# Epist/omnidirectional_collaborative_filtering

Measured on AMD Instinct MI355X. Metric: ratings/sec + masked-RMSE, ML-20M I-AutoRec at 1/2/4/8 MI355X, higher is better.
Workload: dtype f16

## Files before the change

omnidirectional_collaborative_filtering_amd/csrc/ocf_gemm.hip:

```cpp
#include <algorithm>
#include <cstdlib>
#include <type_traits>

#include "ocf_epilogues.h"
#include "ocf_internal.h"
#include "ocf_optim_ws.h"
#include "ocf_rows.h"

using namespace ocf;

namespace {

template <typename CT, bool ACOL, bool BCOL, typename BGT, class Epi, bool SPA = false>
void launch(const OcfGemmArgs& g, const typename Epi::Params& ep, hipStream_t s) {
  using Cfg = GemmCfg<CT, ACOL, BCOL, CT, BGT>;
  constexpr int LDS = std::max(Cfg::OPER_LDS, Epi::LDS_NEED);
  static_assert(LDS <= 160 * 1024, "LDS budget");
  GemmShape sh;
  sh.A = g.A; sh.B = g.B; sh.lda = g.lda; sh.ldb = g.ldb;
  sh.M = g.M; sh.N = g.N; sh.K = g.K; sh.order = g.order;
  sh.a_nt = g.a_nt != 0; sh.b_nt = g.b_nt != 0;
  sh.b_blk = g.b_blocked != 0;
  if (sh.b_blk)
    OCF_CHECK(sizeof(BGT) == 2 && g.ldb % 64 == 0, "ocf_gemm: blocked B needs a 16-bit compute-dtype B and ldb % 64 == 0");
// ... 169 lines not shown
        OCF_CHECK(g.h_dtype == OCF_F32 || g.h_dtype == OCF_BF16, "ocf_gemm GRAD: fp32 or bf16 gradient output");
        EpiGradStore::Params p{g.out, g.ld_out, g.opt.gscale, g.h_dtype == OCF_BF16 ? 1 : 0};
        if constexpr (ACOL) {
          if (g.a_sparse) {
            launch<CT, ACOL, BCOL, CT, EpiGradStore, true>(g, p, s);
            return;
          }
        }
        launch<CT, ACOL, BCOL, CT, EpiGradStore>(g, p, s);
        return;
      }
      break;
    default:
      break;
  }
  throw std::runtime_error("ocf_gemm: epilogue " + std::to_string(g.epi) + " not instantiated for layout a_col=" +
                           std::to_string(ACOL) + " b_col=" + std::to_string(BCOL) + " b_dtype=" +
                           std::to_string(g.b_dtype));
}

template <typename CT, bool ACOL, bool BCOL>
void dispatch_layout(const OcfGemmArgs& g, hipStream_t s) {
  const bool weight_b = g.epi == OCF_EPI_SLAB || g.epi == OCF_EPI_BIAS_ACT || g.epi == OCF_EPI_PREDICT ||
                        g.epi == OCF_EPI_MASKED_MSE || g.epi == OCF_EPI_GRAD_ACT;
  if (weight_b && g.b_dtype == OCF_F32) return dispatch_epi<CT, ACOL, BCOL, float>(g, s);
  OCF_CHECK(g.b_dtype == g.compute_dtype, weight_b ? "ocf_gemm: weight B must be fp32 or the compute dtype"
                                                   : "ocf_gemm: OPTIM/GRAD take B in the compute dtype");
  dispatch_epi<CT, ACOL, BCOL, CT>(g, s);
}


template <typename CT>
void dispatch(const OcfGemmArgs& g, hipStream_t s) {
  if (!g.a_col && g.b_col) dispatch_layout<CT, false, true>(g, s);
  else if (!g.a_col && !g.b_col) dispatch_layout<CT, false, false>(g, s);
  else if (g.a_col && g.b_col) dispatch_layout<CT, true, true>(g, s);
  else throw std::runtime_error("ocf_gemm: layout A[K][M] x B[N][K] not instantiated");
}

}

extern "C" int ocf_set_tuning(const char* key, int value, int* previous) {
  OCF_TRY_BEGIN
  const std::string k = key ? key : "";
  if (k == "optim_rows") {
    if (previous) *previous = g_optim_rows;
    g_optim_rows = value ? 1 : 0;
  } else if (k == "rows_long") {
    if (previous) *previous = g_rows_long;
    g_rows_long = value < 0 ? -1 : (value ? 1 : 0);
  } else if (k == "rows_dual") {
    if (previous) *previous = g_rows_dual;
    g_rows_dual = value ? 1 : 0;
  } else if (k == "rows_dual_parts") {
    if (previous) *previous = g_rows_dual_parts;
    OCF_CHECK(value >= 0 && value <= 64, "ocf_set_tuning: rows_dual_parts 0 (by size) or 1..64");
    g_rows_dual_parts = value;
  } else if (k == "rows_dual_pf") {
    if (previous) *previous = g_rows_dual_pf;
    g_rows_dual_pf = value < 0 ? -1 : value ? 1 : 0;
  } else if (k == "rows_dual_large") {
    if (previous) *previous = g_rows_dual_large;
    g_rows_dual_large = value ? 1 : 0;
  } else if (k == "rows_dual_count") {
    if (previous) *previous = g_rows_dual_count;
    g_rows_dual_count = 0;
  } else if (k == "rows_small_waves") {
    if (previous) *previous = g_rows_small_waves;
    g_rows_small_waves = value;
  } else if (k == "optim_ws") {
    if (previous) *previous = optim_ws_on() ? 1 : 0;
    g_optim_ws = value ? 1 : 0;
  } else if (k == "pair_wait_polls") {
    if (previous) *previous = g_pair_wait_polls;
    OCF_CHECK(value > 0, "ocf_set_tuning: pair_wait_polls > 0");
    g_pair_wait_polls = value;
  } else if (k == "encdec_max_polls") {
    if (previous) *previous = g_encdec_max_polls;
    OCF_CHECK(value != 0, "ocf_set_tuning: encdec_max_polls != 0");
    g_encdec_max_polls = value;
  } else if (k == "encdec_rowres") {
    if (previous) *previous = g_encdec_rowres;
    if (value >= 0) g_encdec_rowres = value ? 1 : 0;
  } else if (k == "mlp_max_polls") {
    if (previous) *previous = g_mlp_max_polls;
    OCF_CHECK(value != 0, "ocf_set_tuning: mlp_max_polls != 0");
    g_mlp_max_polls = value;
  } else if (k == "enc_tiles_pack") {
    if (previous) *previous = g_enc_tiles_pack;
    g_enc_tiles_pack = value ? 1 : 0;
  } else if (k == "optim_ws_max_k") {
    if (previous) *previous = g_optim_ws_max_k;
    g_optim_ws_max_k = value;
  } else {
    throw std::runtime_error("ocf_set_tuning: unknown key '" + k + "'");
  }
  OCF_TRY_END
}

namespace {
void check_gemm(const OcfGemmArgs& g) {
  OCF_CHECK((g.A || g.a_sparse) && g.B, "ocf_gemm: null operand");
  OCF_CHECK(g.M > 0 && g.N > 0 && g.K > 0, "ocf_gemm: empty shape");
  OCF_CHECK(g.M % GT_BM == 0 && g.N % GT_BN == 0, "ocf_gemm: M and N must be multiples of 128");
  const int bk = g.compute_dtype == OCF_F32 ? 32 : 64;
  OCF_CHECK(g.K % bk == 0, "ocf_gemm: K must be a multiple of 64 (f16/bf16) or 32 (f32)");
  OCF_CHECK(g.a_dtype == g.compute_dtype, "ocf_gemm: A must be in the compute dtype");
  OCF_CHECK(g.lda % 8 == 0 && g.ldb % 8 == 0, "ocf_gemm: leading dimensions must be multiples of 8");
  OCF_CHECK(g.splits >= 1, "ocf_gemm: splits >= 1");
  OCF_CHECK(g.splits == 1 || g.epi == OCF_EPI_SLAB, "ocf_gemm: split-K only with the SLAB epilogue");
  if (g.a_sparse) {
    OCF_CHECK(g.a_col && (g.epi == OCF_EPI_OPTIM || g.epi == OCF_EPI_GRAD),
              "ocf_gemm: sparse A only for OPTIM / GRAD with a_col = 1");
    OCF_CHECK(g.sp_rows && g.sp_rp && g.sp_tptr && g.sp_col && g.sp_lidx && g.sp_lboff && g.sp_vals &&
                  g.sp_ntiles * GT_BM >= g.M && g.sp_krows <= g.K,
              "ocf_gemm: sparse A descriptor incomplete");
  }
  OCF_CHECK(!(g.cb_p || g.jb_part || g.js_sp) || (g.epi == OCF_EPI_OPTIM && g.a_col),
            "ocf_gemm: folded jobs only with OPTIM on [K][M] A");
  OCF_CHECK(!g.cb_p || g.sp_colsum, "ocf_gemm: cb_p needs sp_colsum");
  OCF_CHECK(!g.jb_part || g.jb_p, "ocf_gemm: jb_part needs jb_p");
  OCF_CHECK(!g.js_sp || g.js_out, "ocf_gemm: js_sp needs js_out");
}

}

extern "C" int ocf_gemm(const OcfGemmArgs* args, void* stream) {
  OCF_TRY_BEGIN
  const OcfGemmArgs& g = *args;
  check_gemm(g);
  hipStream_t s = (hipStream_t)stream;
  switch (g.compute_dtype) {
    case OCF_F16: dispatch<_Float16>(g, s); break;
    case OCF_BF16: dispatch<__bf16>(g, s); break;
    case OCF_F32: dispatch<float>(g, s); break;
    default: throw std::runtime_error("ocf_gemm: bad compute dtype");
  }
  OCF_TRY_END
}

extern "C" int ocf_gemm_pair(const OcfGemmArgs* a, const OcfGemmArgs* b, OcfPairSync* sync, void* stream) {
  OCF_TRY_BEGIN
  OCF_CHECK(a && b, "ocf_gemm_pair: null arguments");
  OCF_CHECK(!sync || sync->word, "ocf_gemm_pair: OcfPairSync without a device word");
  check_gemm(*a);
  check_gemm(*b);
  hipStream_t s = (hipStream_t)stream;
  bool done = false;
  if (sync && a->compute_dtype == b->compute_dtype) {
    switch (a->compute_dtype) {
      case OCF_F16: done = launch_rows_pair<_Float16>(*a, *b, *sync, s); break;
      case OCF_BF16: done = launch_rows_pair<__bf16>(*a, *b, *sync, s); break;
      case OCF_F32: done = launch_rows_pair<float>(*a, *b, *sync, s); break;
      default: break;
    }
  }
  if (!done) {
    OCF_CHECK(ocf_gemm(a, stream) == 0, ocf_last_error());
    OCF_CHECK(ocf_gemm(b, stream) == 0, ocf_last_error());
  }
  OCF_TRY_END
}

extern "C" int ocf_train_step_rows(const OcfRowStepArgs* a, void* stream) {
  OCF_TRY_BEGIN
  OCF_CHECK(a != nullptr, "ocf_train_step_rows: null arguments");
// ... 32 lines not shown
```

omnidirectional_collaborative_filtering_amd/csrc/ocf_internal.h:

```cpp
#pragma once
#include <exception>
#include <stdexcept>
#include <string>

#include "../../include/ocf.h"
#include "ocf_common.h"

namespace ocf {
using ScatterArgs = OcfScatterArgs;
void set_error(const std::string& msg);
uint32_t* async_error_word();
void check_async_errors();
extern int g_mlp_max_polls;
extern int g_encdec_max_polls;
extern int g_encdec_rowres;
bool rank_rowres_enc(const OcfGatherArgs& e, const OcfRowsReduceArgs& r, hipStream_t s);
bool rank_rowres_dec(const OcfBiasActArgs& hb, const OcfGatherArgs& d, const OcfRowsReduceArgs& r, hipStream_t s);
extern int g_enc_tiles_pack;
uint32_t* encdec_gate_word();
uint32_t encdec_generation();
uint32_t next_encdec_generation();
}

#define OCF_TRY_BEGIN try { ocf::check_async_errors();
#define OCF_TRY_END                                       \
  return 0;                                               \
  }                                                       \
  catch (const std::exception& e) {                       \
    ocf::set_error(e.what());                             \
    return 1;                                             \
  }

#define OCF_CHECK(cond, msg)                              \
  do {                                                    \
    if (!(cond)) throw std::runtime_error(msg);           \
  } while (0)

#define OCF_HIP(expr)                                                               \
  do {                                                                              \
    hipError_t _e = (expr);                                                         \
    if (_e != hipSuccess)                                                           \
      throw std::runtime_error(std::string("HIP error: ") + hipGetErrorString(_e) + \
                               " at " __FILE__ ":" + std::to_string(__LINE__));     \
  } while (0)
```

omnidirectional_collaborative_filtering_amd/csrc/ocf_sparse.hip:

```cpp
#include <algorithm>
#include <cstdlib>

#include "ocf_epilogues.h"
#include "ocf_internal.h"

namespace ocf {

#ifndef OCF_RG_THREADS
#define OCF_RG_THREADS 256
#endif
constexpr int RG_THREADS = OCF_RG_THREADS;
constexpr int RG_MAX_H = 512;
#ifndef OCF_RG_U
#define OCF_RG_U 4
#endif
constexpr int RG_U = OCF_RG_U;
#ifndef OCF_RG_UE
#define OCF_RG_UE 4
#endif
constexpr int RG_UE = OCF_RG_UE;
#ifndef OCF_RG_UD
#define OCF_RG_UD 4
#endif
constexpr int RG_UD = OCF_RG_UD;
// ... 364 lines not shown
        float f[E];
        unpack_piece<WT>(w[u][i], f);
#pragma unroll
        for (int k = 0; k < E; ++k) d0 += hv[i * E + k] * f[k];
      }
      dot[u] = d0;
    }
#pragma unroll
    for (int off = G / 2; off > 0; off >>= 1)
#pragma unroll
      for (int u = 0; u < RG_UD; ++u) dot[u] += __shfl_xor(dot[u], off, G);
#pragma unroll
    for (int u = 0; u < RG_UD; ++u) {
      const int ju = j + u * NG;
      if (ju >= j1) break;
      float d = 0.f;
      if (lv[u]) {
        const float yh = m * (dot[u] + bn[u]);
        const float err = yh - tc[u];
        d = err * m;
        if (l == 0) {
          sse += err * err;
          sae += fabsf(err);
          cnt += (tc[u] + yh != 0.f) ? 1.f : 0.f;
          if (a.d_out) store_ct(a.d_out, a.d_dtype, (int64_t)b * a.ld_d + nc[u], d);
        }
      }
      if (l == 0 && a.delta_e) a.delta_e[lb + ju] = d;
#pragma unroll
      for (int i = 0; i < PPL; ++i) {
        float f[E];
        unpack_piece<WT>(w[u][i], f);
#pragma unroll
        for (int k = 0; k < E; ++k) acc[i * E + k] += d * f[k];
      }
    }
  }
  if (l == 0) {
    st[grp][0] = sse;
    st[grp][1] = sae;
    st[grp][2] = cnt;
  }
  const bool solo = fold && jr.row_cptr[b + 1] - jr.row_cptr[b] == 1;
  float own[RG_XPT];
  reduce_groups<G, V, E, PPL>(acc, red, a.part, c, a.H, grp, l, fold, solo, own);
  float own_st = 0.f;
  if (threadIdx.x < 3) {
    float v = 0.f;
    for (int g = 0; g < NG; ++g) v += st[g][threadIdx.x];
    own_st = v;
    if (solo) {
    } else if (fold) {
      st_sc1(a.chunk_stats, (int64_t)c * 4 + threadIdx.x, v);
    } else {
      a.chunk_stats[(int64_t)c * 4 + threadIdx.x] = v;
    }
  }
  if (fold) dec_row_tail(a, jr, b, a_sh, mk_sh, a.enc_part != nullptr, solo, own, own_st, enc_arrive);
}

template <typename WT, typename HT, int G, int PPL>
__global__ void __launch_bounds__(RG_THREADS) gather_decoder_kernel(OcfGatherArgs a, OcfRowsReduceArgs jr) {
  __shared__ float red[(RG_THREADS / G) * RG_MAX_H];
  decoder_chunk<WT, HT, G, PPL>(a, jr, blockIdx.x, blockIdx.x == 0, red, EncDecSync{});
}

template <typename WT, typename HT, int G, int PPL>
__global__ void __launch_bounds__(RG_THREADS) gather_encdec_kernel(OcfGatherArgs e, OcfGatherArgs d,
                                                                   OcfRowsReduceArgs jr, EncDecSync sy) {
  __shared__ float red[(RG_THREADS / G) * RG_MAX_H];
  const int bx = blockIdx.x;
  if (bx < e.n_chunks) encoder_chunk<WT, G, PPL, RG_UE>(e, bx, red, sy.enc_arrive);
  else decoder_chunk<WT, HT, G, PPL>(d, jr, bx - e.n_chunks, bx == e.n_chunks, red, sy);
}

#ifndef OCF_RR_UD
#define OCF_RR_UD 2
#endif
#ifndef OCF_RR_UE
#define OCF_RR_UE 4
#endif
constexpr int RR_UE = OCF_RR_UE;
constexpr int RR_UD = OCF_RR_UD;

enum { RR_FULL = 0,
       RR_ENC_RAW = 1,
       RR_DEC_RAW = 2 };

template <int G, int V, int E, int PPL>
__device__ __forceinline__ void rr_wave_sums(float (&acc)[V], float (*red)[RG_MAX_H], int l, int lane, int w) {
#pragma unroll
  for (int off = G; off < 64; off <<= 1)
#pragma unroll
    for (int k = 0; k < V; ++k) acc[k] += __shfl_xor(acc[k], off, 64);
  if (lane < G) {
#pragma unroll
    for (int i = 0; i < PPL; ++i)
#pragma unroll
      for (int k = 0; k < E; ++k) red[w][(l + G * i) * E + k] = acc[i * E + k];
  }
}
__device__ __forceinline__ void rr_lds_barrier() { asm volatile("s_waitcnt lgkmcnt(0)\n\ts_barrier" ::: "memory"); }
template <int NW>
__device__ __forceinline__ float rr_row_sum(const float (*red)[RG_MAX_H], int x) {
  float s0 = 0.f, s1 = 0.f;
#pragma unroll
  for (int w = 0; w < NW; w += 2) {
    s0 += red[w][x];
    s1 += red[w + 1][x];
  }
  return s0 + s1;
}
__device__ __forceinline__ float rr_sum_slabs(const float* s, int splits, int64_t sstride) {
  float v0 = 0.f, v1 = 0.f, v2 = 0.f, v3 = 0.f;
  int k = 0;
  for (; k + 4 <= splits; k += 4) {
    v0 += s[(int64_t)(k + 0) * sstride];
    v1 += s[(int64_t)(k + 1) * sstride];
    v2 += s[(int64_t)(k + 2) * sstride];
    v3 += s[(int64_t)(k + 3) * sstride];
  }
  for (; k < splits; ++k) v0 += s[(int64_t)k * sstride];
  return (v0 + v1) + (v2 + v3);
}

template <typename WT, typename HT, int G, int PPL, int T, int MODE>
__global__ void __launch_bounds__(T) gather_rowres_kernel(OcfGatherArgs e, OcfGatherArgs d, OcfRowsReduceArgs r,
                                                          OcfBiasActArgs hb) {
  constexpr int E = EPc<WT>::v;
  constexpr int V = PPL * E;
  constexpr int NG = T / G;
  constexpr int NW = T / 64;
  constexpr int XPT = (RG_MAX_H + T - 1) / T;
  __shared__ float red[NW][RG_MAX_H];
  __shared__ float h_sh[RG_MAX_H];
  __shared__ float a_sh[RG_MAX_H];
  __shared__ uint8_t mk_sh[RG_MAX_H];
  __shared__ float st_sh[NG][3];
  const int b = blockIdx.x, tid = threadIdx.x, lane = tid & 63, w = tid >> 6;
  const int grp = tid / G, l = tid % G;
  const OcfGatherArgs& q = MODE == RR_ENC_RAW ? e : d;
  const int H = q.H;
  const int64_t rb = (int64_t)b * H;
  if (MODE == RR_FULL && d.zero_word && b == 0 && tid == 0)
    __hip_atomic_store(d.zero_word, 0ull, __ATOMIC_RELAXED, __HIP_MEMORY_SCOPE_AGENT);
  const int row = b < r.B ? q.rows[b] : -1;
  const int64_t lb = b < r.B ? q.lboff[b] : 0;
  const int n_e = row >= 0 ? (int)(q.lboff[b + 1] - lb) : 0;
  if (n_e == 0 && MODE != RR_DEC_RAW) {
    for (int x = tid; x < H; x += T) {
      if (MODE == RR_FULL) {
        store_ct(r.h_out, r.h_dtype, rb + x, 0.f);
        if (r.db_part) r.db_part[rb + x] = 0.f;
      } else {
        r.out[rb + x] = 0.f;
      }
    }
    if (MODE == RR_FULL) {
      if (tid < 4) r.stats_part[(int64_t)b * 4 + tid] = 0.f;
      if (tid == 0 && r.row_sse) r.row_sse[b] = 0.f;
    }
    return;
  }
  const int64_t s = n_e > 0 ? q.rp[row] : 0;
  if constexpr (MODE != RR_DEC_RAW) {
    const WT* W = reinterpret_cast<const WT*>(e.W);
// ... 131 lines not shown
        tc[u] = t[u];
      }
      idx_d(j + NG * RR_UD);
      float dot[RR_UD];
#pragma unroll
      for (int u = 0; u < RR_UD; ++u) dot[u] = 0.f;
#pragma unroll
      for (int i = 0; i < PPL; ++i) {
        float hh[E];
#pragma unroll
        for (int k = 0; k < E; ++k) hh[k] = h_sh[(l + G * i) * E + k];
#pragma unroll
        for (int u = 0; u < RR_UD; ++u) {
          float f[E];
          unpack_piece<WT>(wv[u][i], f);
#pragma unroll
          for (int k = 0; k < E; ++k) dot[u] += hh[k] * f[k];
        }
      }
#pragma unroll
      for (int off = G / 2; off > 0; off >>= 1)
#pragma unroll
        for (int u = 0; u < RR_UD; ++u) dot[u] += __shfl_xor(dot[u], off, G);
#pragma unroll
      for (int u = 0; u < RR_UD; ++u) {
        const int ju = j + u * NG;
        if (ju >= n_e) break;
        float dl = 0.f;
        if (lv[u]) {
          const float yh = m * (dot[u] + bn[u]);
          const float err = yh - tc[u];
          dl = err * m;
          if (l == 0) {
            sse += err * err;
            sae += fabsf(err);
            cnt += (tc[u] + yh != 0.f) ? 1.f : 0.f;
            if (d.d_out) store_ct(d.d_out, d.d_dtype, (int64_t)b * d.ld_d + nc[u], dl);
          }
        }
        if (l == 0 && d.delta_e) d.delta_e[lb + ju] = dl;
#pragma unroll
        for (int i = 0; i < PPL; ++i) {
          float f[E];
          unpack_piece<WT>(wv[u][i], f);
#pragma unroll
          for (int k = 0; k < E; ++k) acc[i * E + k] += dl * f[k];
        }
      }
      load_d();
    }
    if (l == 0) {
      st_sh[grp][0] = sse;
      st_sh[grp][1] = sae;
      st_sh[grp][2] = cnt;
    }
    __syncthreads();
    rr_wave_sums<G, V, E, PPL>(acc, red, l, lane, w);
  }
  __syncthreads();
  for (int x = tid; x < H; x += T) {
    const float v = rr_row_sum<NW>(red, x);
    if constexpr (MODE == RR_DEC_RAW) {
      r.out[rb + x] = v;
    } else {
      float dv = 0.f;
      if (x < r.n_real) {
        dv = v;
        if (r.keep < 1.f && r.mask_in) dv = dv * ((float)mk_sh[x] / r.keep);
        dv = dv * act_grad(r.act, a_sh[x]);
      }
      store_ct(r.h_out, r.h_dtype, rb + x, dv);
      if (r.db_part) r.db_part[rb + x] = dv * r.gscale;
    }
  }
  if (tid < 4) {
    float v = 0.f;
    if (tid < 3)
      for (int g = 0; g < NG; ++g) v += st_sh[g][tid];
    r.stats_part[(int64_t)b * 4 + tid] = v;
    if (tid == 0 && r.row_sse) r.row_sse[b] = v;
  }
}

__global__ void __launch_bounds__(256) rows_reduce_kernel(OcfRowsReduceArgs a) {
  const int b = blockIdx.x;
  const bool real = b < a.B;
  const int c0 = real ? a.row_cptr[b] : 0, c1 = real ? a.row_cptr[b + 1] : 0;
  for (int x = threadIdx.x; x < a.H; x += blockDim.x) {
    float v = 0.f;
    for (int c = c0; c < c1; c += 8) {
      float q[8];
#pragma unroll
      for (int k = 0; k < 8; ++k) q[k] = c + k < c1 ? a.part[(int64_t)(c + k) * a.H + x] : 0.f;
#pragma unroll
      for (int k = 0; k < 8; ++k)
        if (c + k < c1) v += q[k];
    }
    if (a.mode == OCF_REDUCE_RAW) {
      a.out[(int64_t)b * a.H + x] = v;
    } else if (a.mode == OCF_REDUCE_BIAS_ACT) {
      BiasActParams p;
      p.bias = a.bias; p.act = a.act; p.keep = a.keep; p.seed = a.seed; p.stream = a.stream;
      p.mask_in = a.mask_in; p.mask_out = a.mask_out; p.a_out = a.a_out; p.h_out = a.h_out;
      p.h_dtype = a.h_dtype; p.ld = a.H; p.m_real = a.B; p.n_real = a.n_real;
      bias_act_store(p, b, x, v);
    } else {
      GradActParams p;
      p.a = a.a_in; p.mask = a.mask_in; p.keep = a.keep; p.act = a.act; p.d_out = a.h_out; p.d_dtype = a.h_dtype;
      p.ld = a.H; p.db_part = nullptr; p.gscale = a.gscale; p.m_real = a.B; p.n_real = a.n_real;
      const float d = grad_act_value(p, b, x, v);
      store_ct(a.h_out, a.h_dtype, (int64_t)b * a.H + x, d);
      if (a.db_part) a.db_part[(int64_t)b * a.H + x] = d * a.gscale;
    }
  }
  if (a.chunk_stats && threadIdx.x < 4) {
    float v = 0.f;
    if (threadIdx.x < 3)
      for (int c = c0; c < c1; c += 8) {
        float q[8];
#pragma unroll
        for (int k = 0; k < 8; ++k) q[k] = c + k < c1 ? a.chunk_stats[(int64_t)(c + k) * 4 + threadIdx.x] : 0.f;
#pragma unroll
        for (int k = 0; k < 8; ++k)
          if (c + k < c1) v += q[k];
      }
    a.stats_part[(int64_t)b * 4 + threadIdx.x] = v;
    if (threadIdx.x == 0 && a.row_sse) a.row_sse[b] = v;
  }
}

template <typename WT> bool gather_shape(int H, int& G, int& ppl) {
  const int pieces = H / EPc<WT>::v;
  constexpr int gmax = 32;
  for (int g : {64, 32, 16})
    if (g <= gmax && pieces % g == 0 && pieces / g <= 4) {
      G = g;
      ppl = pieces / g;
      return true;
    }
  for (int g : {64, 32, 16})
    if (pieces % g == 0) {
      G = g;
      ppl = pieces / g;
      return ppl <= 3;
    }
  return false;
}

template <template <int, int> class L>
void by_shape(int G, int ppl, const OcfGatherArgs& a, hipStream_t s) {
  if (G == 64 && ppl == 1) L<64, 1>::go(a, s);
  else if (G == 64 && ppl == 2) L<64, 2>::go(a, s);
  else if (G == 32 && ppl == 1) L<32, 1>::go(a, s);
  else if (G == 32 && ppl == 2) L<32, 2>::go(a, s);
  else if (G == 16 && ppl == 4) L<16, 4>::go(a, s);
  else if (G == 32 && ppl == 4) L<32, 4>::go(a, s);
  else if (G == 32 && ppl == 3) L<32, 3>::go(a, s);
  else if (G == 16 && ppl == 1) L<16, 1>::go(a, s);
  else if (G == 16 && ppl == 3) L<16, 3>::go(a, s);
  else throw std::runtime_error("row gather: unsupported H / weight dtype combination");
}

template <typename WT> struct Enc {
  template <int G, int P> struct L {
    static void go(const OcfGatherArgs& a, hipStream_t s) {
      hipLaunchKernelGGL((gather_encoder_kernel<WT, G, P>), dim3(a.n_chunks), dim3(RG_THREADS), 0, s, a);
    }
  };
};
template <typename WT, typename HT> struct Dec {
  template <int G, int P> struct L {
    static void go(const OcfGatherArgs& a, hipStream_t s) {
      OcfRowsReduceArgs r{};
      if (a.jr && a.row_arrive) r = *a.jr;
      hipLaunchKernelGGL((gather_decoder_kernel<WT, HT, G, P>), dim3(a.n_chunks), dim3(RG_THREADS), 0, s, a, r);
    }
  };
};

template <typename WT, typename HT>
void launch_encdec(int G, int ppl, const OcfGatherArgs& e, const OcfGatherArgs& d, const EncDecSync& sy, hipStream_t s) {
  OcfRowsReduceArgs r = *d.jr;
  const dim3 grid(e.n_chunks + d.n_chunks), blk(RG_THREADS);
#define OCF_ED(GG, PP) hipLaunchKernelGGL((gather_encdec_kernel<WT, HT, GG, PP>), grid, blk, 0, s, e, d, r, sy)
  if (G == 64 && ppl == 1) OCF_ED(64, 1);
  else if (G == 64 && ppl == 2) OCF_ED(64, 2);
  else if (G == 32 && ppl == 1) OCF_ED(32, 1);
  else if (G == 32 && ppl == 2) OCF_ED(32, 2);
  else if (G == 16 && ppl == 4) OCF_ED(16, 4);
  else if (G == 32 && ppl == 4) OCF_ED(32, 4);
  else if (G == 32 && ppl == 3) OCF_ED(32, 3);
  else if (G == 16 && ppl == 1) OCF_ED(16, 1);
  else if (G == 16 && ppl == 3) OCF_ED(16, 3);
  else throw std::runtime_error("row gather: unsupported H / weight dtype combination");
#undef OCF_ED
}

template <typename WT, typename HT, int T, int MODE>
void launch_rowres_t(int G, int ppl, const OcfGatherArgs& e, const OcfGatherArgs& d, const OcfRowsReduceArgs& r,
                     const OcfBiasActArgs& hb, hipStream_t s) {
  const dim3 grid(r.Bp), blk(T);
#define OCF_RR(GG, PP) hipLaunchKernelGGL((gather_rowres_kernel<WT, HT, GG, PP, T, MODE>), grid, blk, 0, s, e, d, r, hb)
  if (G == 32 && ppl == 2) OCF_RR(32, 2);
  else if (G == 64 && ppl == 2) OCF_RR(64, 2);
  else if (G == 64 && ppl == 1) OCF_RR(64, 1);
  else if (G == 32 && ppl == 1) OCF_RR(32, 1);
  else if (G == 16 && ppl == 1) OCF_RR(16, 1);
  else throw std::runtime_error("row gather (row-resident): unsupported H / weight dtype combination");
#undef OCF_RR
}
template <int MODE>
void launch_rowres(int dtype, int H, int T, const OcfGatherArgs& e, const OcfGatherArgs& d,
                   const OcfRowsReduceArgs& r, const OcfBiasActArgs& hb, hipStream_t s) {
  int G, ppl;
  if (dtype == OCF_F32) {
    G = 64;
    ppl = H / 256;
  } else if (!(dtype == OCF_F16 ? gather_shape<_Float16>(H, G, ppl) : gather_shape<__bf16>(H, G, ppl))) {
    throw std::runtime_error("row gather (row-resident): unsupported H");
  }
  auto go = [&](auto wt) {
    using WT = decltype(wt);
    if (T == 256) launch_rowres_t<WT, WT, 256, MODE>(G, ppl, e, d, r, hb, s);
    else launch_rowres_t<WT, WT, 1024, MODE>(G, ppl, e, d, r, hb, s);
  };
  if (dtype == OCF_F32) go(float{});
  else if (dtype == OCF_F16) go(_Float16{});
  else go(__bf16{});
}
bool rowres_shape_ok(int dtype, int H) { return dtype == OCF_F32 ? H % 256 == 0 : H != 384; }

void check_gather(const OcfGatherArgs& a, const char* who) {
  OCF_CHECK(a.rows && a.rp && a.col && a.lboff && a.ch_row && a.ch_j0 && a.ch_j1 && a.W && a.part,
            std::string(who) + ": null pointer");
  OCF_CHECK(a.H > 0 && a.H <= RG_MAX_H && a.H % 128 == 0, std::string(who) + ": H must be a multiple of 128, <= 512");
  OCF_CHECK(a.w_dtype == OCF_F32 || a.w_dtype == OCF_F16 || a.w_dtype == OCF_BF16, std::string(who) + ": w_dtype");
  OCF_CHECK(!a.w_blocked || a.w_dtype != OCF_F32, std::string(who) + ": blocked weights are 16-bit");
  OCF_CHECK(a.ldw >= a.H && a.ldw % 8 == 0, std::string(who) + ": ldw");
}

template <typename WT> void shape_or_throw(const OcfGatherArgs& a, int& G, int& ppl) {
  if (!gather_shape<WT>(a.H, G, ppl)) throw std::runtime_error("row gather: unsupported H " + std::to_string(a.H));
}

}

using namespace ocf;

extern "C" int ocf_gather_encoder(const OcfGatherArgs* args, void* stream) {
  OCF_TRY_BEGIN
  const OcfGatherArgs& a = *args;
  check_gather(a, "ocf_gather_encoder");
  OCF_CHECK(a.xval != nullptr, "ocf_gather_encoder: xval required");
  if (a.n_chunks == 0) return 0;
  hipStream_t s = (hipStream_t)stream;
  int G, ppl;
  if (a.w_dtype == OCF_F32) { shape_or_throw<float>(a, G, ppl); by_shape<Enc<float>::L>(G, ppl, a, s); }
  else if (a.w_dtype == OCF_F16) { shape_or_throw<_Float16>(a, G, ppl); by_shape<Enc<_Float16>::L>(G, ppl, a, s); }
  else { shape_or_throw<__bf16>(a, G, ppl); by_shape<Enc<__bf16>::L>(G, ppl, a, s); }
  OCF_HIP(hipGetLastError());
  OCF_TRY_END
}

extern "C" int ocf_gather_decoder(const OcfGatherArgs* args, void* stream) {
  OCF_TRY_BEGIN
  const OcfGatherArgs& a = *args;
  check_gather(a, "ocf_gather_decoder");
  OCF_CHECK(a.flag && a.val && a.h && a.bias && a.chunk_stats, "ocf_gather_decoder: flag/val/h/bias/chunk_stats required");
  OCF_CHECK(a.h_dtype == a.w_dtype, "ocf_gather_decoder: h and W must share the compute dtype");
  OCF_CHECK(!a.enc_part || (a.enc_cptr && a.bias_h && (a.keep >= 1.f || a.mask_out) && a.a_out),
            "ocf_gather_decoder: enc_part needs enc_cptr, bias_h, a_out and (with dropout) mask_out");
  OCF_CHECK(!a.jr == !a.row_arrive, "ocf_gather_decoder: jr and row_arrive go together");
  if (a.jr) {
    const OcfRowsReduceArgs& r = *a.jr;
    OCF_CHECK(r.mode == OCF_REDUCE_GRAD_ACT && r.part == a.part && r.chunk_stats == a.chunk_stats && r.H == a.H &&
                  r.row_cptr && r.h_out && r.a_in && r.stats_part && r.B <= r.Bp && (r.keep >= 1.f || r.mask_in),
              "ocf_gather_decoder: jr must be OCF_REDUCE_GRAD_ACT over this launch's part / chunk_stats (same H) "
              "with row_cptr, h_out, a_in, stats_part and (with dropout) mask_in");
  }
  if (a.n_chunks == 0) {
    OCF_CHECK(!a.jr, "ocf_gather_decoder: a folded row reduction needs at least one chunk");
    return 0;
  }
  hipStream_t s = (hipStream_t)stream;
  int G, ppl;
  if (a.w_dtype == OCF_F32) { shape_or_throw<float>(a, G, ppl); by_shape<Dec<float, float>::L>(G, ppl, a, s); }
  else if (a.w_dtype == OCF_F16) {
    shape_or_throw<_Float16>(a, G, ppl);
    by_shape<Dec<_Float16, _Float16>::L>(G, ppl, a, s);
  } else {
    shape_or_throw<__bf16>(a, G, ppl);
    by_shape<Dec<__bf16, __bf16>::L>(G, ppl, a, s);
  }
  OCF_HIP(hipGetLastError());
  OCF_TRY_END
}

namespace ocf {
int g_encdec_max_polls = 1 << 22;
int g_encdec_rowres = [] {
  const char* v = std::getenv("OCF_ENCDEC_ROWRES");
  return v ? std::atoi(v) : 1;
}();
}

extern "C" int ocf_gather_encdec(const OcfGatherArgs* enc, const OcfGatherArgs* dec, uint32_t* enc_arrive,
                                 void* stream) {
  OCF_TRY_BEGIN
  OCF_CHECK(enc && dec && enc_arrive, "ocf_gather_encdec: null arguments");
  const OcfGatherArgs& e = *enc;
  const OcfGatherArgs& d = *dec;
  check_gather(e, "ocf_gather_encdec (encoder)");
  check_gather(d, "ocf_gather_encdec (decoder)");
  OCF_CHECK(e.xval != nullptr, "ocf_gather_encdec: xval required");
  OCF_CHECK(d.flag && d.val && d.h && d.bias && d.chunk_stats, "ocf_gather_encdec: flag/val/h/bias/chunk_stats required");
  OCF_CHECK(d.h_dtype == d.w_dtype && e.w_dtype == d.w_dtype && e.H == d.H, "ocf_gather_encdec: one dtype and H");
  OCF_CHECK(d.enc_part == e.part && d.enc_cptr && d.bias_h && (d.keep >= 1.f || d.mask_out) && d.a_out,
            "ocf_gather_encdec: dec.enc_part must be enc.part, with enc_cptr, bias_h, a_out (and mask_out)");
  OCF_CHECK(d.jr && d.row_arrive, "ocf_gather_encdec: the decoder's folded row reduction (jr, row_arrive) is required");
  OCF_CHECK(e.ch_row == d.ch_row && e.ch_j0 == d.ch_j0 && e.ch_j1 == d.ch_j1 && e.n_chunks == d.n_chunks &&
                e.rows == d.rows && e.lboff == d.lboff && e.rp == d.rp,
            "ocf_gather_encdec: the encoder and the decoder must share the batch's chunk table");
  const OcfRowsReduceArgs& r = *d.jr;
  OCF_CHECK(r.mode == OCF_REDUCE_GRAD_ACT && r.part == d.part && r.chunk_stats == d.chunk_stats && r.H == d.H &&
                r.row_cptr && r.h_out && r.a_in && r.stats_part && r.B <= r.Bp && (r.keep >= 1.f || r.mask_in),
            "ocf_gather_encdec: jr must be OCF_REDUCE_GRAD_ACT over the decoder's part / chunk_stats");
  if (d.n_chunks == 0) return 0;
  hipStream_t s = (hipStream_t)stream;
  int G, ppl;
  if (g_encdec_rowres && r.Bp > 0 && rowres_shape_ok(d.w_dtype, d.H)) {
    launch_rowres<RR_FULL>(d.w_dtype, d.H, 1024, e, d, r, OcfBiasActArgs{}, s);
    OCF_HIP(hipGetLastError());
    return 0;
  }
  EncDecSync sy{enc_arrive, async_error_word(), nullptr, 0, g_encdec_max_polls};
  sy.gen = next_encdec_generation();
  sy.gate = encdec_gate_word();
  if (d.w_dtype == OCF_F32) { shape_or_throw<float>(d, G, ppl); launch_encdec<float, float>(G, ppl, e, d, sy, s); }
  else if (d.w_dtype == OCF_F16) { shape_or_throw<_Float16>(d, G, ppl); launch_encdec<_Float16, _Float16>(G, ppl, e, d, sy, s); }
  else { shape_or_throw<__bf16>(d, G, ppl); launch_encdec<__bf16, __bf16>(G, ppl, e, d, sy, s); }
  OCF_HIP(hipGetLastError());
  OCF_TRY_END
}

namespace ocf {
bool rank_rowres_enc(const OcfGatherArgs& e, const OcfRowsReduceArgs& r, hipStream_t s) {
  if (!(g_encdec_rowres && rowres_shape_ok(e.w_dtype, e.H) && r.mode == OCF_REDUCE_RAW && r.out && r.H == e.H &&
        e.xval && r.Bp > 0 && r.B <= r.Bp && e.n_chunks > 0))
    return false;
  check_gather(e, "ocf_rank_step (row-resident encoder)");
  const int T = e.n_chunks <= 2 * r.B ? 256 : 1024;
  launch_rowres<RR_ENC_RAW>(e.w_dtype, e.H, T, e, e, r, OcfBiasActArgs{}, s);
  OCF_HIP(hipGetLastError());
  return true;
}
bool rank_rowres_dec(const OcfBiasActArgs& hb, const OcfGatherArgs& d, const OcfRowsReduceArgs& r, hipStream_t s) {
  if (!(g_encdec_rowres && rowres_shape_ok(d.w_dtype, d.H) && r.mode == OCF_REDUCE_RAW && r.out && r.H == d.H &&
        r.stats_part && r.Bp > 0 && r.B <= r.Bp && d.n_chunks > 0 && !d.enc_part && !d.jr && d.flag && d.val &&
        d.bias && hb.slabs && hb.splits >= 1 && hb.M == r.Bp && hb.N == d.H && hb.ld >= d.H && hb.bias &&
        d.h_dtype == d.w_dtype && hb.h_dtype == d.w_dtype && (hb.keep >= 1.f || hb.mask_out || hb.mask_in)))
    return false;
  check_gather(d, "ocf_rank_step (row-resident decoder)");
  const int T = d.n_chunks <= 2 * r.B ? 256 : 1024;
  launch_rowres<RR_DEC_RAW>(d.w_dtype, d.H, T, d, d, r, hb, s);
  OCF_HIP(hipGetLastError());
  return true;
}
}

extern "C" int ocf_rows_reduce(const OcfRowsReduceArgs* args, void* stream) {
  OCF_TRY_BEGIN
  const OcfRowsReduceArgs& a = *args;
  OCF_CHECK(a.part && a.row_cptr && a.H > 0 && a.B <= a.Bp, "ocf_rows_reduce: bad arguments");
  OCF_CHECK(a.mode != OCF_REDUCE_RAW || a.out, "ocf_rows_reduce: RAW needs out");
  OCF_CHECK(a.mode == OCF_REDUCE_RAW || a.h_out, "ocf_rows_reduce: BIAS_ACT / GRAD_ACT need h_out");
  OCF_CHECK(!a.chunk_stats || a.stats_part, "ocf_rows_reduce: chunk_stats needs stats_part");
  if (a.Bp == 0) return 0;
  hipLaunchKernelGGL(rows_reduce_kernel, dim3(a.Bp), dim3(256), 0, (hipStream_t)stream, a);
  OCF_HIP(hipGetLastError());
  OCF_TRY_END
}

namespace ocf {
__global__ void __launch_bounds__(256) colsum_kernel(const void* d, int dtype, int64_t ld, int B, int N, float gscale,
                                                     float* out) {
  const int n = blockIdx.x * 256 + threadIdx.x;
  if (n >= N) return;
  float s0 = 0.f, s1 = 0.f;
  int b = 0;
  for (; b + 2 <= B; b += 2) {
    s0 += load_ct(d, dtype, (int64_t)b * ld + n);
    s1 += load_ct(d, dtype, (int64_t)(b + 1) * ld + n);
  }
  if (b < B) s0 += load_ct(d, dtype, (int64_t)b * ld + n);
  out[n] = (s0 + s1) * gscale;
}
}

extern "C" int ocf_colsum(const void* d, int dtype, int64_t ld, int B, int N, float gscale, float* out, void* stream) {
  OCF_TRY_BEGIN
  OCF_CHECK(d && out && ld >= N, "ocf_colsum: bad arguments");
  if (N == 0) return 0;
  hipLaunchKernelGGL(colsum_kernel, dim3((N + 255) / 256), dim3(256), 0, (hipStream_t)stream, d, dtype, ld, B, N, gscale,
                     out);
  OCF_HIP(hipGetLastError());
  OCF_TRY_END
}

namespace ocf {

struct TbSeg {
  int64_t e0;
  int n;
  int64_t lb;
// ... 747 lines not shown
```

Before: 465.1 million.

## Add LDS-queued row-resident encdec kernel with async global-to-LDS weight prefetch

Adds a new row-resident encoder/decoder kernel that streams weight rows into a per-wave LDS ring buffer using global_load_lds_dwordx4 direct loads, S slots deep. This hides gather latency by keeping several row fetches in flight, and it prefetches the decoder's first rows while the encoder reduction runs. The kernel is gated to H==512 with 2-8 chunks per row and falls back to the register-based kernel otherwise. It uses much more LDS, which lowers occupancy, and relies on inline asm that manipulates m0. The tile size of the fallback path also becomes a compile-time option.

```diff
diff --git a/omnidirectional_collaborative_filtering_amd/csrc/ocf_gemm.hip b/omnidirectional_collaborative_filtering_amd/csrc/ocf_gemm.hip
--- a/omnidirectional_collaborative_filtering_amd/csrc/ocf_gemm.hip
+++ b/omnidirectional_collaborative_filtering_amd/csrc/ocf_gemm.hip
@@ -275,6 +275,16 @@
   } else if (k == "encdec_rowres") {
     if (previous) *previous = g_encdec_rowres;
     if (value >= 0) g_encdec_rowres = value ? 1 : 0;
+  } else if (k == "rowres_queue") {
+    if (previous) *previous = g_rowres_queue;
+    OCF_CHECK(value == 0 || value == 1, "ocf_set_tuning: rowres_queue 0 (registers) or 1 (LDS queue)");
+    g_rowres_queue = value;
+  } else if (k == "rowres_queue_gate") {
+    if (previous) *previous = g_rowres_queue_gate;
+    g_rowres_queue_gate = value ? 1 : 0;
+  } else if (k == "rowres_queue_count") {
+    if (previous) *previous = g_rowres_queue_count;
+    g_rowres_queue_count = 0;
   } else if (k == "mlp_max_polls") {
     if (previous) *previous = g_mlp_max_polls;
     OCF_CHECK(value != 0, "ocf_set_tuning: mlp_max_polls != 0");
diff --git a/omnidirectional_collaborative_filtering_amd/csrc/ocf_internal.h b/omnidirectional_collaborative_filtering_amd/csrc/ocf_internal.h
--- a/omnidirectional_collaborative_filtering_amd/csrc/ocf_internal.h
+++ b/omnidirectional_collaborative_filtering_amd/csrc/ocf_internal.h
@@ -14,6 +14,9 @@
 extern int g_mlp_max_polls;
 extern int g_encdec_max_polls;
 extern int g_encdec_rowres;
+extern int g_rowres_queue_gate;
+extern int g_rowres_queue_count;
+extern int g_rowres_queue;
 bool rank_rowres_enc(const OcfGatherArgs& e, const OcfRowsReduceArgs& r, hipStream_t s);
 bool rank_rowres_dec(const OcfBiasActArgs& hb, const OcfGatherArgs& d, const OcfRowsReduceArgs& r, hipStream_t s);
 extern int g_enc_tiles_pack;
diff --git a/omnidirectional_collaborative_filtering_amd/csrc/ocf_sparse.hip b/omnidirectional_collaborative_filtering_amd/csrc/ocf_sparse.hip
--- a/omnidirectional_collaborative_filtering_amd/csrc/ocf_sparse.hip
+++ b/omnidirectional_collaborative_filtering_amd/csrc/ocf_sparse.hip
@@ -470,6 +470,9 @@
 #endif
 constexpr int RR_UE = OCF_RR_UE;
 constexpr int RR_UD = OCF_RR_UD;
+#ifndef OCF_RR_T
+#define OCF_RR_T 1024
+#endif
 
 enum { RR_FULL = 0,
        RR_ENC_RAW = 1,
@@ -767,6 +770,300 @@
   }
 }
 
+#ifndef OCF_RQ_S
+#define OCF_RQ_S 3
+#endif
+constexpr int RQ_S = OCF_RQ_S;
+constexpr int RQ_T = 1024;
+
+template <int G, int PPL, int S> struct RqLds {
+  static constexpr int NW = RQ_T / 64, NG = RQ_T / G;
+  static constexpr int SLOT = PPL * 1024;
+  static constexpr int ring = 0;
+  static constexpr int red = ring + NW * S * SLOT;
+  static constexpr int h = red + NW * RG_MAX_H * 4;
+  static constexpr int a = h + RG_MAX_H * 4;
+  static constexpr int erow = a + RG_MAX_H * 4;
+  static constexpr int xv = erow + RQ_T * 4;
+  static constexpr int drow = xv + RQ_T * 4;
+  static constexpr int val = drow + RQ_T * 4;
+  static constexpr int bn = val + RQ_T * 4;
+  static constexpr int dl = xv;
+  static constexpr int st = bn + RQ_T * 4;
+  static constexpr int mk = st + NG * 3 * 4;
+  static constexpr int fl = mk + RG_MAX_H;
+  static constexpr int bytes = fl + RQ_T;
+  static_assert(bytes <= 160 * 1024, "row-resident queue: LDS");
+};
+
+__device__ __forceinline__ void rq_dma16(const void* src, uint32_t dst) {
+  uint32_t keep;
+  asm volatile("s_mov_b32 %0, m0\n\ts_mov_b32 m0, %2\n\ts_nop 0\n\tglobal_load_lds_dwordx4 %1, off\n\ts_mov_b32 m0, %0"
+               : "=&s"(keep)
+               : "v"(src), "s"(dst)
+               : "memory");
+}
+template <int N> __device__ __forceinline__ void rq_wait_vm() { asm volatile("s_waitcnt vmcnt(%0)" ::"n"(N) : "memory"); }
+__device__ __forceinline__ void rq_wait_lds() { asm volatile("s_waitcnt lgkmcnt(0)" ::: "memory"); }
+
+template <typename WT, int G, int PPL, int S>
+__global__ void __launch_bounds__(RQ_T) gather_rowres_queue_kernel(OcfGatherArgs e, OcfGatherArgs d,
+                                                                   OcfRowsReduceArgs r) {
+  static_assert(sizeof(WT) == 2, "row-resident queue: 16-bit weights");
+  constexpr int T = RQ_T;
+  constexpr int E = EPc<WT>::v;
+  constexpr int V = PPL * E;
+  constexpr int NG = T / G;
+  constexpr int NW = T / 64;
+  constexpr int GPW = 64 / G;
+  using L = RqLds<G, PPL, S>;
+  extern __shared__ __attribute__((aligned(16))) unsigned char rq_lds[];
+  float(*red)[RG_MAX_H] = reinterpret_cast<float(*)[RG_MAX_H]>(rq_lds + L::red);
+  float* h_sh = reinterpret_cast<float*>(rq_lds + L::h);
+  float* a_sh = reinterpret_cast<float*>(rq_lds + L::a);
+  int* erow_sh = reinterpret_cast<int*>(rq_lds + L::erow);
+  int* drow_sh = reinterpret_cast<int*>(rq_lds + L::drow);
+  float* xv_sh = reinterpret_cast<float*>(rq_lds + L::xv);
+  float* val_sh = reinterpret_cast<float*>(rq_lds + L::val);
+  float* bn_sh = reinterpret_cast<float*>(rq_lds + L::bn);
+  float* dl_sh = reinterpret_cast<float*>(rq_lds + L::dl);
+  float(*st_sh)[3] = reinterpret_cast<float(*)[3]>(rq_lds + L::st);
+  uint8_t* mk_sh = rq_lds + L::mk;
+  uint8_t* fl_sh = rq_lds + L::fl;
+  const int b = blockIdx.x, tid = threadIdx.x, lane = tid & 63;
+  const int w = __builtin_amdgcn_readfirstlane(tid >> 6);
+  const int grp = tid / G, l = tid % G;
+  const int H = d.H;
+  const int64_t rb = (int64_t)b * H;
+  if (d.zero_word && b == 0 && tid == 0)
+    __hip_atomic_store(d.zero_word, 0ull, __ATOMIC_RELAXED, __HIP_MEMORY_SCOPE_AGENT);
+  const int row = b < r.B ? d.rows[b] : -1;
+  const int64_t lb = b < r.B ? d.lboff[b] : 0;
+  const int n_e = row >= 0 ? (int)(d.lboff[b + 1] - lb) : 0;
+  if (n_e == 0) {
+    for (int x = tid; x < H; x += T) {
+      store_ct(r.h_out, r.h_dtype, rb + x, 0.f);
+      if (r.db_part) r.db_part[rb + x] = 0.f;
+    }
+    if (tid < 4) r.stats_part[(int64_t)b * 4 + tid] = 0.f;
+    if (tid == 0 && r.row_sse) r.row_sse[b] = 0.f;
+    return;
+  }
+  const int64_t s = d.rp[row];
+  const bool lvx = tid < H && b < d.m_real && tid < d.n_real;
+  const float bh = lvx ? d.bias_h[tid] : 0.f;
+  const int n_tiles = (n_e + T - 1) / T;
+  auto stage = [&](int t, bool enc, bool dec) {
+    const int j = t * T + tid;
+    const bool in = j < n_e;
+    const int c = in ? d.col[s + j] : 0;
+    if (enc) {
+      const float x = in ? e.xval[lb + j] : 0.f;
+      xv_sh[tid] = x;
+      erow_sh[tid] = x != 0.f ? c : 0;
+    }
+    if (dec) {
+      const uint8_t f = in ? d.flag[lb + j] : (uint8_t)0;
+      fl_sh[tid] = f;
+      drow_sh[tid] = f ? c : 0;
+      val_sh[tid] = in ? d.val[s + j] : 0.f;
+      bn_sh[tid] = d.bias[f ? c : 0];
+    }
+  };
+  const uint32_t ring0 = __builtin_amdgcn_readfirstlane(
+      (uint32_t)(size_t)(__attribute__((address_space(3))) unsigned char*)rq_lds + L::ring + w * S * L::SLOT);
+  const unsigned char* ring_rd = rq_lds + L::ring + w * S * L::SLOT + lane * 16;
+  int pce[PPL], pcd[PPL];
+#pragma unroll
+  for (int i = 0; i < PPL; ++i) {
+    const int hc = (l + G * i) * E;
+    pce[i] = e.w_blocked ? ((hc >> 6) << 13) + (hc & 63) * 2 : hc * 2;
+    pcd[i] = d.w_blocked ? ((hc >> 6) << 13) + (hc & 63) * 2 : hc * 2;
+  }
+  struct RowAt { int sh, mk; int64_t hi; };
+  auto row_at = [](const OcfGatherArgs& g) {
+    return g.w_blocked ? RowAt{6, 63, (int64_t)(g.ldw >> 6) << 13} : RowAt{0, 0, (int64_t)g.ldw * 2};
+  };
+  const RowAt rae = row_at(e), rad = row_at(d);
+  auto rowoff = [](const RowAt& ra, int n) -> int64_t { return (int64_t)(n >> ra.sh) * ra.hi + (n & ra.mk) * 128; };
+  auto request = [&](const char* Wb, int64_t ro, const int (&pc)[PPL], int sl) {
+#pragma unroll
+    for (int i = 0; i < PPL; ++i) rq_dma16(Wb + ro + pc[i], ring0 + (uint32_t)((sl * PPL + i) * 1024));
+  };
+  auto read_slot = [&](int sl, uint4 (&wv)[PPL]) {
+#pragma unroll
+    for (int i = 0; i < PPL; ++i) wv[i] = *reinterpret_cast<const uint4*>(ring_rd + (sl * PPL + i) * 1024);
+  };
+  auto wave_iters = [&](int nt) { return nt > w * GPW ? (nt - w * GPW + NG - 1) / NG : 0; };
+  {
+    const char* We = reinterpret_cast<const char*>(e.W);
+    float acc[V];
+#pragma unroll
+    for (int k = 0; k < V; ++k) acc[k] = 0.f;
+    for (int t = 0; t < n_tiles; ++t) {
+      if (t > 0) rr_lds_barrier();
+      stage(t, true, n_tiles == 1);
+      __syncthreads();
+      const int nt = min(T, n_e - t * T);
+      const int nk = wave_iters(nt);
+#pragma unroll
+      for (int k = 0; k < S; ++k)
+        if (k < nk) request(We, rowoff(rae, erow_sh[grp + k * NG]), pce, k);
+      int sl = 0;
+      for (int k = 0; k < nk; ++k) {
+        if (k + S <= nk) rq_wait_vm<(S - 1) * PPL>();
+        else rq_wait_vm<0>();
+        uint4 wv[PPL];
+        read_slot(sl, wv);
+        const float xc = xv_sh[grp + k * NG];
+        const bool more = k + S < nk;
+        const int nn = erow_sh[grp + min(k + S, nk - 1) * NG];
+        rq_wait_lds();
+        if (more) request(We, rowoff(rae, nn), pce, sl);
+        sl = sl + 1 == S ? 0 : sl + 1;
+#pragma unroll
+        for (int i = 0; i < PPL; ++i) {
+          if (xc == 0.f) wv[i] = make_uint4(0, 0, 0, 0);
+          float f[E];
+          unpack_piece<WT>(wv[i], f);
+#pragma unroll
+          for (int k2 = 0; k2 < E; ++k2) acc[i * E + k2] += xc * f[k2];
+        }
+      }
+    }
+    if (n_tiles > 1) {
+      rr_lds_barrier();
+      stage(0, false, true);
+      __syncthreads();
+    }
+    const char* Wd0 = reinterpret_cast<const char*>(d.W);
+    const int nk0 = wave_iters(min(T, n_e));
+#pragma unroll
+    for (int k = 0; k < S; ++k)
+      if (k < nk0) request(Wd0, rowoff(rad, drow_sh[grp + k * NG]), pcd, k);
+    rr_wave_sums<G, V, E, PPL>(acc, red, l, lane, w);
+  }
+  rr_lds_barrier();
+  if (tid < H) {
+    const int x = tid;
+    const int64_t ix = (int64_t)b * H + x;
+    const float v = rr_row_sum<NW>(red, x);
+    const float av = lvx ? act_apply(d.act, v + bh) : 0.f;
+    float hvx = av;
+    a_sh[x] = av;
+    if (d.keep < 1.f) {
+      const uint8_t mk = (uint8_t)floorf(d.keep + philox_uniform(d.seed, d.stream, (uint64_t)ix));
+      hvx = (av / d.keep) * (float)mk;
+      if (d.mask_out) d.mask_out[ix] = mk;
+      mk_sh[x] = mk;
+    }
+    if (d.a_out) d.a_out[ix] = av;
+    if (d.h) store_ct(const_cast<void*>(d.h), d.h_dtype, ix, hvx);
+    h_sh[x] = (float)CvtT<WT>::to(hvx);
+  }
+  rr_lds_barrier();
+  {
+    const char* Wd = reinterpret_cast<const char*>(d.W);
+    const float m = d.aux;
+    float hv[V];
+#pragma unroll
+    for (int i = 0; i < PPL; ++i)
+#pragma unroll
+      for (int k = 0; k < E; ++k) hv[i * E + k] = h_sh[(l + G * i) * E + k];
+    float acc[V];
+#pragma unroll
+    for (int k = 0; k < V; ++k) acc[k] = 0.f;
+    float sse = 0.f, sae = 0.f, cnt = 0.f;
+    for (int t = 0; t < n_tiles; ++t) {
+      const int nt = min(T, n_e - t * T);
+      const int nk = wave_iters(nt);
+      if (t > 0) {
+        rr_lds_barrier();
+        stage(t, false, true);
+        __syncthreads();
+#pragma unroll
+        for (int k = 0; k < S; ++k)
+          if (k < nk) request(Wd, rowoff(rad, drow_sh[grp + k * NG]), pcd, k);
+      }
+      int sl = 0;
+      for (int k = 0; k < nk; ++k) {
+        if (k + S <= nk) rq_wait_vm<(S - 1) * PPL>();
+        else rq_wait_vm<0>();
+        uint4 wv[PPL];
+        read_slot(sl, wv);
+        const int jl = grp + k * NG;
+        const bool lv = fl_sh[jl] != 0;
+        const float tc = val_sh[jl], bnv = bn_sh[jl];
+        const bool more = k + S < nk;
+        const int nn = drow_sh[grp + min(k + S, nk - 1) * NG];
+        rq_wait_lds();
+        if (more) request(Wd, rowoff(rad, nn), pcd, sl);
+        sl = sl + 1 == S ? 0 : sl + 1;
+        float dot = 0.f;
+#pragma unroll
+        for (int i = 0; i < PPL; ++i) {
+          float f[E];
+          unpack_piece<WT>(wv[i], f);
+#pragma unroll
+          for (int k2 = 0; k2 < E; ++k2) dot += hv[i * E + k2] * f[k2];
+        }
+#pragma unroll
+        for (int off = G / 2; off > 0; off >>= 1) dot += __shfl_xor(dot, off, G);
+        float dl = 0.f;
+        if (lv) {
+          const float yh = m * (dot + bnv);
+          const float err = yh - tc;
+          dl = err * m;
+          if (l == 0) {
+            sse += err * err;
+            sae += fabsf(err);
+            cnt += (tc + yh != 0.f) ? 1.f : 0.f;
+          }
+        }
+        if (l == 0) dl_sh[jl] = dl;
+#pragma unroll
+        for (int i = 0; i < PPL; ++i) {
+          float f[E];
+          unpack_piece<WT>(wv[i], f);
+#pragma unroll
+          for (int k2 = 0; k2 < E; ++k2) acc[i * E + k2] += dl * f[k2];
+        }
+      }
+      if (d.delta_e) {
+        rr_lds_barrier();
+        if (tid < nt) d.delta_e[lb + (int64_t)t * T + tid] = dl_sh[tid];
+      }
+    }
+    if (l == 0) {
+      st_sh[grp][0] = sse;
+      st_sh[grp][1] = sae;
+      st_sh[grp][2] = cnt;
+    }
+    __syncthreads();
+    rr_wave_sums<G, V, E, PPL>(acc, red, l, lane, w);
+  }
+  __syncthreads();
+  if (tid < H) {
+    const int x = tid;
+    const float v = rr_row_sum<NW>(red, x);
+    float dv = 0.f;
+    if (x < r.n_real) {
+      dv = v;
+      if (r.keep < 1.f && r.mask_in) dv = dv * ((float)mk_sh[x] / r.keep);
+      dv = dv * act_grad(r.act, a_sh[x]);
+    }
+    store_ct(r.h_out, r.h_dtype, rb + x, dv);
+    if (r.db_part) r.db_part[rb + x] = dv * r.gscale;
+  }
+  if (tid < 4) {
+    float v = 0.f;
+    if (tid < 3)
+      for (int g = 0; g < NG; ++g) v += st_sh[g][tid];
+    r.stats_part[(int64_t)b * 4 + tid] = v;
+    if (tid == 0 && r.row_sse) r.row_sse[b] = v;
+  }
+}
+
 __global__ void __launch_bounds__(256) rows_reduce_kernel(OcfRowsReduceArgs a) {
   const int b = blockIdx.x;
   const bool real = b < a.B;
@@ -907,11 +1204,40 @@
   auto go = [&](auto wt) {
     using WT = decltype(wt);
     if (T == 256) launch_rowres_t<WT, WT, 256, MODE>(G, ppl, e, d, r, hb, s);
+#if OCF_RR_T == 512
+    else if (T == 512) launch_rowres_t<WT, WT, 512, MODE>(G, ppl, e, d, r, hb, s);
+#endif
     else launch_rowres_t<WT, WT, 1024, MODE>(G, ppl, e, d, r, hb, s);
   };
   if (dtype == OCF_F32) go(float{});
   else if (dtype == OCF_F16) go(_Float16{});
   else go(__bf16{});
+}
+template <typename WT>
+bool launch_rowres_queue_t(int G, int ppl, const OcfGatherArgs& e, const OcfGatherArgs& d, const OcfRowsReduceArgs& r,
+                           hipStream_t s) {
+  const dim3 grid(r.Bp), blk(RQ_T);
+#define OCF_RQ(GG, PP)                                                                                              \
+  do {                                                                                                              \
+    constexpr int bytes = RqLds<GG, PP, RQ_S>::bytes;                                                               \
+    static const bool lds_attr =                                                                                    \
+        hipFuncSetAttribute((const void*)gather_rowres_queue_kernel<WT, GG, PP, RQ_S>,                              \
+                            hipFuncAttributeMaxDynamicSharedMemorySize, bytes) == hipSuccess;                       \
+    OCF_CHECK(lds_attr, "row gather (row-resident queue): cannot raise the dynamic LDS limit");                     \
+    hipLaunchKernelGGL((gather_rowres_queue_kernel<WT, GG, PP, RQ_S>), grid, blk, bytes, s, e, d, r);               \
+  } while (0)
+  if (G == 32 && ppl == 2) OCF_RQ(32, 2);
+  else if (G == 32 && ppl == 1) OCF_RQ(32, 1);
+  else if (G == 16 && ppl == 1) OCF_RQ(16, 1);
+  else return false;
+#undef OCF_RQ
+  return true;
+}
+bool launch_rowres_queue(const OcfGatherArgs& e, const OcfGatherArgs& d, const OcfRowsReduceArgs& r, hipStream_t s) {
+  if (d.w_dtype == OCF_F32 || d.d_out || e.col != d.col) return false;
+  int G, ppl;
+  if (d.w_dtype == OCF_F16) return gather_shape<_Float16>(d.H, G, ppl) && launch_rowres_queue_t<_Float16>(G, ppl, e, d, r, s);
+  return gather_shape<__bf16>(d.H, G, ppl) && launch_rowres_queue_t<__bf16>(G, ppl, e, d, r, s);
 }
 bool rowres_shape_ok(int dtype, int H) { return dtype == OCF_F32 ? H % 256 == 0 : H != 384; }
 
@@ -987,6 +1313,12 @@
   const char* v = std::getenv("OCF_ENCDEC_ROWRES");
   return v ? std::atoi(v) : 1;
 }();
+int g_rowres_queue = 1;
+int g_rowres_queue_count = 0;
+int g_rowres_queue_gate = 1;
+bool rowres_queue_gate(const OcfGatherArgs& d, const OcfRowsReduceArgs& r) {
+  return d.H == 512 && d.n_chunks >= 2 * (int64_t)r.B && d.n_chunks <= 8 * (int64_t)r.B;
+}
 }
 
 extern "C" int ocf_gather_encdec(const OcfGatherArgs* enc, const OcfGatherArgs* dec, uint32_t* enc_arrive,
@@ -1014,7 +1346,9 @@
   hipStream_t s = (hipStream_t)stream;
   int G, ppl;
   if (g_encdec_rowres && r.Bp > 0 && rowres_shape_ok(d.w_dtype, d.H)) {
-    launch_rowres<RR_FULL>(d.w_dtype, d.H, 1024, e, d, r, OcfBiasActArgs{}, s);
+    if (g_rowres_queue && (!g_rowres_queue_gate || rowres_queue_gate(d, r)) && launch_rowres_queue(e, d, r, s))
+      ++g_rowres_queue_count;
+    else launch_rowres<RR_FULL>(d.w_dtype, d.H, OCF_RR_T, e, d, r, OcfBiasActArgs{}, s);
     OCF_HIP(hipGetLastError());
     return 0;
   }
```

Result: faster. 476.5 million, median of 6 (+2.4%).
